# HikariTJU/LD

Hardware: AMD Instinct MI355X
Metric: images/sec (1333x800) GFocal-R50<-R101 LD train step (higher is better)
Workload: dtype f32

## Files before the change

ld_amd/csrc/conv.hip:

```cpp
#include <hip/hip_runtime.h>
#include <type_traits>
#include <stdio.h>
#include <stdlib.h>

#include <mutex>
#include <string>
#include <unordered_map>
#include <vector>

#include "conv_common.h"
#include "conv_tune.h"

namespace {

template <int BM, int BNT, int BKT, int MODE, int KG, int WVM, int WVN>
__global__ __launch_bounds__(64 * WVM * WVN * KG) void conv_igemm_kernel(ConvK a) {
  constexpr int NT = 64 * WVM * WVN;
  constexpr int WM = BM / WVM, WN = BNT / WVN;
  constexpr int TM = WM / 32, TN = WN / 32;
  constexpr int A_PER = BKT * BM / NT;
  constexpr int B_PER = BKT * BNT / NT;
  static_assert(A_PER >= 1 && B_PER >= 1, "tile too small");
  constexpr int NBUF = 2;
  constexpr int GROUP_LDS = NBUF * BKT * (BM + BNT);
  constexpr int NACC = TM * TN * 16;
  static_assert(KG == 1 || (KG - 1) * NACC * NT <= KG * GROUP_LDS,
                "split-K reduction does not fit the tile LDS");
  __shared__ float lds[KG * GROUP_LDS + 2 * BM];
  const int kg = __builtin_amdgcn_readfirstlane((int)threadIdx.x / NT);
  float* As = lds + kg * GROUP_LDS;
  float* Bs = As + NBUF * BKT * BM;

  const int t = threadIdx.x % NT, lane = t & 63, wave = t >> 6;
  const int wm = wave / WVN, wn = wave % WVN;
  const int mtiles = (a.Cout + BM - 1) / BM;
  const int tile = xcd_swizzle(blockIdx.x, gridDim.x);
  const int m0 = (tile % mtiles) * BM;
  const int n0 = (tile / mtiles) * BNT;

  const int jb = n0 + (t % BNT);
  const bool jvalid = jb < a.J;
  int bHin = 0, bWin = 0, boff = 0, bh0 = 0, bw0 = 0;
  if (jvalid) {
    const int n = jb / a.Pout, p = jb - n * a.Pout;
    int bl, bho, bwo;
    locate_out(a.g, p, bl, bho, bwo);
    bHin = a.g.lv[bl].Hin;
    bWin = a.g.lv[bl].Win;
    boff = n * a.Cin * a.Pin + a.g.lv[bl].off_in;
    if (MODE == 1) {
      bh0 = bho + a.ch0;
      bw0 = bwo + a.cw0;
    } else {
      bh0 = bho * a.g.stride - a.g.pad;
      bw0 = bwo * a.g.stride - a.g.pad;
    }
  }
  auto tap_off = [&](int kh, int kw, int& off) -> bool {
    const int hi = bh0 + kh, wi = bw0 + kw;
    if (hi < 0 || hi >= bHin || wi < 0 || wi >= bWin) return false;
    off = boff + hi * bWin + wi;
    return true;
  };
  static_assert(BNT >= 64, "B row groups must be wave-uniform");
  const int bk0 = __builtin_amdgcn_readfirstlane((t / BNT) * B_PER);
  const int am = t % BM;
  const bool avalid = (m0 + am) < a.Cout;
  const int ak0s = __builtin_amdgcn_readfirstlane(((wave * 64) / BM) * A_PER);
  const int ak0v = (BM < 64) ? (lane / BM) * A_PER : 0;
  const int ak0 = ak0s + ak0v;

  floatx16 acc[TM][TN];
#pragma unroll
  for (int i = 0; i < TM; ++i)
#pragma unroll
    for (int j = 0; j < TN; ++j)
#pragma unroll
      for (int r = 0; r < 16; ++r) acc[i][j][r] = 0.0f;

  const int Cin = __builtin_amdgcn_readfirstlane(a.Cin);
  const int Cout = __builtin_amdgcn_readfirstlane(a.Cout);
  const int KW = __builtin_amdgcn_readfirstlane(a.KW);
  const int Pin = __builtin_amdgcn_readfirstlane(a.Pin);
  const int ntaps = __builtin_amdgcn_readfirstlane(
      MODE == 1 ? a.nth * a.ntw : a.KH * a.KW);
  const int csteps = (Cin + BKT - 1) / BKT;
  const int ktot = Cin * ntaps;
  const int nsteps = (MODE == 2) ? (ktot + BKT - 1) / BKT : ntaps * csteps;
  float a_st[A_PER], b_st[B_PER];

  const rsrc_t rx = make_rsrc(a.x, a.x_bytes);
  const rsrc_t rw = make_rsrc(a.wt, a.wt_bytes);
  const int Kpad = __builtin_amdgcn_readfirstlane(a.Kpad);
  const unsigned va =
      avalid ? (unsigned)(m0 + am + ak0v * Cout) * 4u : kOOB;
  auto load_tile = [&](int step, float* ra, float* rb) {
    if (MODE == 2) {
      const int k0 = step * BKT;
#pragma unroll
      for (int i = 0; i < A_PER; ++i)
        ra[i] = buf_load(rw, va, (unsigned)(k0 + ak0s + i) * Cout * 4u);
#pragma unroll
      for (int i = 0; i < B_PER; ++i) {
        const int k = k0 + bk0 + i;
        const int ci = min(k / ntaps, Cin - 1);
        const int r = k % ntaps;
        const int kh = r / KW, kw = r - kh * KW;
        int off = 0;
        const bool kb = jvalid && tap_off(kh, kw, off);
        rb[i] = buf_load(rx, kb ? (unsigned)off * 4u : kOOB,
                           (unsigned)ci * Pin * 4u);
      }
      return;
    }
    int tap = step / csteps;
    const int ci0 = (step - tap * csteps) * BKT;
    int kh, kw;
    if (MODE == 1) {
      const int ntw = __builtin_amdgcn_readfirstlane(a.ntw);
      kh = tap / ntw;
      kw = tap - kh * ntw;
      tap = (a.kh0 + 2 * kh) * KW + a.kw0 + 2 * kw;
    } else {
      kh = tap / KW;
      kw = tap - kh * KW;
    }
    int off = 0;
    const bool ok = jvalid && tap_off(kh, kw, off);
    const unsigned vb = ok ? (unsigned)off * 4u : kOOB;
    const unsigned sa = (unsigned)(tap * Kpad + ci0 + ak0s) * Cout * 4u;
#pragma unroll
    for (int i = 0; i < A_PER; ++i)
      ra[i] = buf_load(rw, va, sa + (unsigned)i * Cout * 4u);
#pragma unroll
    for (int i = 0; i < B_PER; ++i) {
      const int row = min(ci0 + bk0 + i, Cin - 1);
      rb[i] = buf_load(rx, vb, (unsigned)row * Pin * 4u);
    }
  };
  auto store_tile = [&](int buf, const float* ra, const float* rb) {
    float* ap = As + buf * BKT * BM + ak0 * BM + am;
#pragma unroll
    for (int i = 0; i < A_PER; ++i) ap[i * BM] = ra[i];
    float* bp = Bs + buf * BKT * BNT + bk0 * BNT + (t % BNT);
#pragma unroll
    for (int i = 0; i < B_PER; ++i) bp[i * BNT] = rb[i];
  };

  const int l31 = lane & 31, lk = lane >> 5;
  constexpr int KP = BKT / 2;
  auto compute = [&](int buf) {
    const float* ap = As + buf * BKT * BM + wm * WM + l31;
    const float* bp = Bs + buf * BKT * BNT + wn * WN + l31;
    float af[2][TM], bf[2][TN];
#pragma unroll
    for (int i = 0; i < TM; ++i) af[0][i] = ap[lk * BM + i * 32];
// ... 37 lines not shown
      for (int i = 0; i < TM; ++i) f0a[i] = ap[lk * BM + i * 32];
#pragma unroll
      for (int j = 0; j < TN; ++j) f0b[j] = bp[lk * BNT + j * 32];
    };
    auto pstep = [&](int buf, bool has_next, const float* wa, const float* wb) {
      const float* ap = As + buf * BKT * BM + wm * WM + l31;
      const float* bp = Bs + buf * BKT * BNT + wn * WN + l31;
      float af[2][TM], bf[2][TN];
#pragma unroll
      for (int i = 0; i < TM; ++i) af[0][i] = f0a[i];
#pragma unroll
      for (int j = 0; j < TN; ++j) bf[0][j] = f0b[j];
#pragma unroll
      for (int kp = 0; kp < KP; ++kp) {
        const int c = kp & 1;
        if (kp + 1 < KP) {
          const int kr = 2 * (kp + 1) + lk;
#pragma unroll
          for (int i = 0; i < TM; ++i) af[c ^ 1][i] = ap[kr * BM + i * 32];
#pragma unroll
          for (int j = 0; j < TN; ++j) bf[c ^ 1][j] = bp[kr * BNT + j * 32];
        }
        if (kp == WPOS && has_next) store_tile(buf ^ 1, wa, wb);
        if (kp == KP - 2) {
          __syncthreads();
          if (has_next) frag0(buf ^ 1);
        }
        __builtin_amdgcn_sched_barrier(0);
#pragma unroll
        for (int i = 0; i < TM; ++i)
#pragma unroll
          for (int j = 0; j < TN; ++j)
            acc[i][j] = __builtin_amdgcn_mfma_f32_32x32x2f32(af[c][i], bf[c][j],
                                                             acc[i][j], 0, 0, 0);
        __builtin_amdgcn_sched_barrier(0);
      }
    };
    load_tile(0, a_st, b_st);
    store_tile(0, a_st, b_st);
    if (nsteps > 1) load_tile(1, a_s2, b_s2);
    __syncthreads();
    frag0(0);
    for (int step = 0; step < nsteps; step += 2) {
      if (step + 2 < nsteps) load_tile(step + 2, a_st, b_st);
      pstep(0, step + 1 < nsteps, a_s2, b_s2);
      if (step + 1 < nsteps) {
        if (step + 3 < nsteps) load_tile(step + 3, a_s2, b_s2);
        pstep(1, step + 2 < nsteps, a_st, b_st);
      }
    }
  } else {
  const int iters = (nsteps + KG - 1) / KG;
  if (kg < nsteps) {
    load_tile(kg, a_st, b_st);
    store_tile(0, a_st, b_st);
  }
  __syncthreads();
  for (int it = 0; it < iters; ++it) {
    const int cur = it & 1;
    const int step = kg + it * KG;
    const bool more = step + KG < nsteps;
    if (more) load_tile(step + KG, a_st, b_st);
    if (step < nsteps) compute(cur);
    if (more) store_tile(cur ^ 1, a_st, b_st);
    __syncthreads();
  }
  }
  __syncthreads();

  float* s_scale = lds + KG * GROUP_LDS;
  float* s_shift = s_scale + BM;
  if (KG > 1 && kg > 0) {
    float* red = lds + (size_t)(kg - 1) * NACC * NT + t;
#pragma unroll
    for (int i = 0; i < TM; ++i)
#pragma unroll
      for (int j = 0; j < TN; ++j)
#pragma unroll
        for (int r = 0; r < 16; ++r)
          red[((i * TN + j) * 16 + r) * NT] = acc[i][j][r];
  }
  if (kg == 0 && t < BM) {
    const int co = m0 + t;
    float sc = 1.0f, sh = 0.0f;
    if (co < a.Cout) {
      if (a.scale) {
        sc = a.scale[co];
        sh = a.shift[co];
      }
      if (a.bias) sh += a.bias[co];
    }
    s_scale[t] = sc;
    s_shift[t] = sh;
  }
  __syncthreads();
  if (KG > 1) {
    if (kg > 0) return;
#pragma unroll
    for (int g = 1; g < KG; ++g) {
      const float* red = lds + (size_t)(g - 1) * NACC * NT + t;
#pragma unroll
      for (int i = 0; i < TM; ++i)
#pragma unroll
        for (int j = 0; j < TN; ++j)
#pragma unroll
          for (int r = 0; r < 16; ++r)
            acc[i][j][r] += red[((i * TN + j) * 16 + r) * NT];
    }
  }
  const bool has_res = a.residual != nullptr;
  const bool relu = a.relu != 0;
#pragma unroll
  for (int j = 0; j < TN; ++j) {
    const int jc = n0 + wn * WN + j * 32 + l31;
    if (jc >= a.J) continue;
    const int n = jc / a.Pout;
    int p = jc - n * a.Pout;
    int prow = a.Pout;
    if (MODE == 1) {
      int l, hc, wc;
      locate_out(a.g, p, l, hc, wc);
      p = a.foff[l] + (2 * hc + a.ph) * a.fW[l] + 2 * wc + a.pw;
      prow = a.Pfull;
    }
    const size_t colbase = (size_t)n * a.Cout * prow + p;
#pragma unroll
    for (int i = 0; i < TM; ++i) {
      const int rbase = wm * WM + i * 32 + 4 * lk;
      float res[16];
      if (has_res) {
#pragma unroll
        for (int r = 0; r < 16; ++r) {
          const int row = rbase + (r & 3) + 8 * (r >> 2);
          res[r] = (m0 + row < a.Cout)
                       ? a.residual[colbase + (size_t)(m0 + row) * prow]
                       : 0.0f;
        }
      }
#pragma unroll
      for (int r = 0; r < 16; ++r) {
        const int row = rbase + (r & 3) + 8 * (r >> 2);
        if (m0 + row >= a.Cout) continue;
        float v = acc[i][j][r] * s_scale[row] + s_shift[row];
        if (MODE == 0 && a.y_raw)
          a.y_raw[colbase + (size_t)(m0 + row) * prow] = acc[i][j][r];
        if (has_res) v += res[r];
        if (relu) v = fmaxf(v, 0.0f);
        a.y[colbase + (size_t)(m0 + row) * prow] = v;
      }
    }
  }
}

template <int TM, int TN, int WVM, int MODE, int D, int OCC, int KS, int DBG = 0>
__global__ __launch_bounds__(256, OCC) void conv_stream_kernel(ConvK a) {
  static_assert(KS == 1 || (KS == 4 && WVM == 1), "KS is 1 or 4");
  static_assert(D * (TM + TN) < 64, "ring exceeds the 6-bit vmcnt counter");
  constexpr int WVN = 4 / WVM;
  constexpr int WM = TM * 32, WN = TN * 32;
  constexpr int BM = KS == 4 ? WM : WVM * WM, BNT = KS == 4 ? WN : WVN * WN;
  __shared__ float red[KS == 4 ? 2 * TM * TN * 16 * 64 : 1];
  const int lane = threadIdx.x & 63;
  const int wave = __builtin_amdgcn_readfirstlane((int)threadIdx.x >> 6);
  const int wm = KS == 4 ? 0 : wave / WVN, wn = KS == 4 ? 0 : wave % WVN;
  const int kslice = KS == 4 ? wave : 0;
  const int l31 = lane & 31, lk = lane >> 5;
  const int mtiles = (a.Cout + BM - 1) / BM;
  const int tile = xcd_swizzle(blockIdx.x, gridDim.x);
  const int m0 = (tile % mtiles) * BM + wm * WM;
  const int n0 = (tile / mtiles) * BNT + wn * WN;
  if (m0 >= a.Cout || n0 >= a.J) return;

  const int Cin = __builtin_amdgcn_readfirstlane(a.Cin);
  const int Cout = __builtin_amdgcn_readfirstlane(a.Cout);
  const int KW = __builtin_amdgcn_readfirstlane(a.KW);
  const int Pin = __builtin_amdgcn_readfirstlane(a.Pin);
  const int Kpad = __builtin_amdgcn_readfirstlane(a.Kpad);
  const int ntw = __builtin_amdgcn_readfirstlane(MODE == 1 ? a.ntw : a.KW);
  const int ntaps = __builtin_amdgcn_readfirstlane(
      MODE == 1 ? a.nth * a.ntw : a.KH * a.KW);

  int bHin[TN], bWin[TN], boff[TN], bh0[TN], bw0[TN];
#pragma unroll
  for (int j = 0; j < TN; ++j) {
    const int jb = n0 + j * 32 + l31;
    bHin[j] = 0;
    bWin[j] = 0;
    boff[j] = 0;
    bh0[j] = 0;
    bw0[j] = 0;
    if (jb < a.J) {
      const int n = jb / a.Pout, p = jb - n * a.Pout;
      int bl, bho, bwo;
      locate_out(a.g, p, bl, bho, bwo);
      bHin[j] = a.g.lv[bl].Hin;
      bWin[j] = a.g.lv[bl].Win;
      boff[j] = n * Cin * Pin + a.g.lv[bl].off_in + lk * Pin;
      if (MODE == 1) {
        bh0[j] = bho + a.ch0;
        bw0[j] = bwo + a.cw0;
      } else {
        bh0[j] = bho * a.g.stride - a.g.pad;
        bw0[j] = bwo * a.g.stride - a.g.pad;
      }
    }
  }
  unsigned va[TM];
#pragma unroll
  for (int i = 0; i < TM; ++i) {
    const int co = m0 + i * 32 + l31;
    va[i] = co < Cout ? (unsigned)(lk * Cout + co) * 4u : kOOB;
  }
  const rsrc_t rx = make_rsrc(a.x, a.x_bytes);
  const rsrc_t rw = make_rsrc(a.wt, a.wt_bytes);

  unsigned vb[TN];
  int wtap = 0;
  auto set_tap = [&](int tap) {
    int kh = tap / ntw, kw = tap - kh * ntw;
    if (MODE == 1) {
      wtap = (a.kh0 + 2 * kh) * KW + a.kw0 + 2 * kw;
    } else {
      wtap = tap;
    }
#pragma unroll
    for (int j = 0; j < TN; ++j) {
      const int hi = bh0[j] + kh, wi = bw0[j] + kw;
      const bool ok = hi >= 0 && hi < bHin[j] && wi >= 0 && wi < bWin[j];
      vb[j] = ok ? (unsigned)(boff[j] + hi * bWin[j] + wi) * 4u : kOOB;
    }
  };
  float ra[D][TM], rb[D][TN];
  auto load_kp = [&](int d, unsigned sa, unsigned sb) {
#pragma unroll
    for (int i = 0; i < TM; ++i) ra[d][i] = buf_load(rw, (DBG & 4) ? kOOB : va[i], sa);
#pragma unroll
    for (int j = 0; j < TN; ++j) rb[d][j] = buf_load(rx, (DBG & 2) ? kOOB : vb[j], sb);
  };

  floatx16 acc[TM][TN];
#pragma unroll
  for (int i = 0; i < TM; ++i)
#pragma unroll
    for (int j = 0; j < TN; ++j)
#pragma unroll
      for (int r = 0; r < 16; ++r) acc[i][j][r] = 0.0f;
  auto mfma_kp = [&](int d) {
#pragma unroll
    for (int i = 0; i < TM; ++i)
#pragma unroll
      for (int j = 0; j < TN; ++j)
        acc[i][j] = __builtin_amdgcn_mfma_f32_32x32x2f32(ra[d][i], rb[d][j],
                                                         acc[i][j], 0, 0, 0);
  };

  const int cchunks = Cin / (2 * D);
  const int nchunks = ntaps * cchunks;
  const int mychunks = nchunks > kslice ? (nchunks - kslice + KS - 1) / KS : 0;
  int ltap = 0, lci = 0;
  auto advance = [&](int n) {
    lci += 2 * D * n;
    const int t0 = ltap;
    while (lci >= Cin) {
      lci -= Cin;
      ++ltap;
    }
    if (ltap != t0 && ltap < ntaps) set_tap(ltap);
  };
  set_tap(0);
  if (KS > 1) advance(kslice);
  if (mychunks > 0) {
    {
      const unsigned sa = (unsigned)(wtap * Kpad + lci) * Cout * 4u;
      const unsigned sb = (unsigned)lci * Pin * 4u;
#pragma unroll
      for (int d = 0; d < D; ++d) {
        load_kp(d, sa + (unsigned)(2 * d) * Cout * 4u,
                sb + (unsigned)(2 * d) * Pin * 4u);
        __builtin_amdgcn_sched_barrier(0);
      }
      advance(KS);
    }
    for (int c = 0; c + 1 < mychunks; ++c) {
      const unsigned sa = (unsigned)(wtap * Kpad + lci) * Cout * 4u;
      const unsigned sb = (unsigned)lci * Pin * 4u;
#pragma unroll
      for (int d = 0; d < D; ++d) {
        mfma_kp(d);
        __builtin_amdgcn_sched_barrier(0);
        if (!(DBG & 1))
          load_kp(d, sa + (unsigned)(2 * d) * Cout * 4u,
                  sb + (unsigned)(2 * d) * Pin * 4u);
        __builtin_amdgcn_sched_barrier(0);
      }
      advance(KS);
    }
#pragma unroll
    for (int d = 0; d < D; ++d) mfma_kp(d);
  }
  if (KS == 4) {
    constexpr int NACC = TM * TN * 16;
    auto put = [&](float* dst) {
#pragma unroll
      for (int i = 0; i < TM; ++i)
#pragma unroll
        for (int j = 0; j < TN; ++j)
#pragma unroll
          for (int r = 0; r < 16; ++r)
            dst[((i * TN + j) * 16 + r) * 64 + lane] = acc[i][j][r];
    };
    auto add = [&](const float* src) {
#pragma unroll
      for (int i = 0; i < TM; ++i)
#pragma unroll
        for (int j = 0; j < TN; ++j)
#pragma unroll
          for (int r = 0; r < 16; ++r)
            acc[i][j][r] += src[((i * TN + j) * 16 + r) * 64 + lane];
    };
    if (wave >= 2) put(red + (size_t)(wave - 2) * NACC * 64);
    __syncthreads();
    if (wave < 2) add(red + (size_t)wave * NACC * 64);
    __syncthreads();
    if (wave == 1) put(red);
    __syncthreads();
    if (wave != 0) return;
    add(red);
  }

  if (DBG & 8) {
    float s = 0.0f;
#pragma unroll
    for (int i = 0; i < TM; ++i)
#pragma unroll
      for (int j = 0; j < TN; ++j)
#pragma unroll
        for (int r = 0; r < 16; ++r) s += acc[i][j][r];
    if (s == 1.2345e-30f) a.y[0] = s;
    return;
  }
  const bool has_res = a.residual != nullptr;
  const bool has_raw = MODE == 0 && a.y_raw != nullptr;
  const bool relu = a.relu != 0;
  const bool has_aff = a.scale != nullptr, has_bias = a.bias != nullptr;
  const int prow = __builtin_amdgcn_readfirstlane(MODE == 1 ? a.Pfull : a.Pout);
  const unsigned ybytes = (unsigned)a.N * (unsigned)Cout * (unsigned)prow * 4u;
  const rsrc_t r_y = make_rsrc(a.y, ybytes);
  const rsrc_t r_raw = make_rsrc(a.y_raw, has_raw ? ybytes : 0u);
  const rsrc_t r_res = make_rsrc(a.residual, has_res ? ybytes : 0u);
  const rsrc_t r_sc = make_rsrc(a.scale, has_aff ? (unsigned)Cout * 4u : 0u);
  const rsrc_t r_sh = make_rsrc(a.shift, has_aff ? (unsigned)Cout * 4u : 0u);
  const rsrc_t r_bi = make_rsrc(a.bias, has_bias ? (unsigned)Cout * 4u : 0u);
  unsigned voff[TN];
#pragma unroll
  for (int j = 0; j < TN; ++j) {
    const int jc = n0 + j * 32 + l31;
    const int n = jc / a.Pout;
    int p = jc - n * a.Pout;
    if (MODE == 1 && jc < a.J) {
      int l, hc, wc;
      locate_out(a.g, p, l, hc, wc);
      p = a.foff[l] + (2 * hc + a.ph) * a.fW[l] + 2 * wc + a.pw;
    }
    voff[j] = jc < a.J ? ((unsigned)(n * Cout + m0 + 4 * lk) * (unsigned)prow + (unsigned)p) * 4u
                       : kOOB;
  }
  const unsigned prow4 = (unsigned)prow * 4u;
  auto run = [&](auto res_c, auto raw_c) {
    constexpr bool RES = decltype(res_c)::value, RAW = decltype(raw_c)::value;
#pragma unroll
    for (int ig = 0; ig < TM * 4; ++ig) {
      const int i = ig >> 2, g = ig & 3;
      const int rl = i * 32 + 8 * g;
      __builtin_amdgcn_sched_barrier(0);
      float sc[4], sh[4], bi[4], rv[TN][4];
#pragma unroll
      for (int e = 0; e < 4; ++e) {
        const unsigned ro = (unsigned)(m0 + 4 * lk + rl + e) * 4u;
        sc[e] = buf_load(r_sc, ro, 0);
        sh[e] = buf_load(r_sh, ro, 0);
        bi[e] = buf_load(r_bi, ro, 0);
      }
      if (RES) {
#pragma unroll
        for (int j = 0; j < TN; ++j)
#pragma unroll
          for (int e = 0; e < 4; ++e) {
            const bool ok = m0 + 4 * lk + rl + e < Cout;
            rv[j][e] = buf_load(r_res, ok ? voff[j] : kOOB, (unsigned)(rl + e) * prow4);
          }
      }
#pragma unroll
      for (int e = 0; e < 4; ++e) {
        const bool ok = m0 + 4 * lk + rl + e < Cout;
        const float scale = has_aff ? sc[e] : 1.0f;
        const float shift = sh[e] + bi[e];
        const unsigned so = (unsigned)(rl + e) * prow4;
#pragma unroll
        for (int j = 0; j < TN; ++j) {
          const int r = 4 * g + e;
          const unsigned vo = ok ? voff[j] : kOOB;
          const float av = acc[i][j][r];
          float v = av * scale + shift;
          if (RAW)
            __builtin_amdgcn_raw_buffer_store_b32(__builtin_bit_cast(unsigned, av), r_raw,
                                                  vo, so, 0);
          if (RES) v += rv[j][e];
          v = relu ? fmaxf(v, 0.0f) : v;
          __builtin_amdgcn_raw_buffer_store_b32(__builtin_bit_cast(unsigned, v), r_y, vo,
                                                so, 0);
        }
      }
    }
  };
  if (has_res) {
    if (has_raw) run(std::true_type{}, std::true_type{});
    else run(std::true_type{}, std::false_type{});
  } else {
    if (has_raw) run(std::false_type{}, std::true_type{});
    else run(std::false_type{}, std::false_type{});
  }
}

template <int VEC>
struct VecF;
template <>
struct VecF<2> { typedef float T __attribute__((ext_vector_type(2))); };
template <>
struct VecF<4> { typedef float T __attribute__((ext_vector_type(4))); };

template <int VEC>
__device__ __forceinline__ typename VecF<VEC>::T buf_load_vec(rsrc_t r, unsigned voff,
                                                             unsigned soff) {
  typedef typename VecF<VEC>::T V;
  if constexpr (VEC == 2)
    return __builtin_bit_cast(V, __builtin_amdgcn_raw_buffer_load_b64(r, voff, soff, 0));
  else
    return __builtin_bit_cast(V, __builtin_amdgcn_raw_buffer_load_b128(r, voff, soff, 0));
}

template <int TM, int VEC, int WVM, int D>
__global__ __launch_bounds__(256, 2) void conv1x1_vec_kernel(ConvK a) {
  static_assert(D * (TM + 1) < 64, "ring exceeds the 6-bit vmcnt counter");
  typedef typename VecF<VEC>::T V;
  constexpr int WVN = 4 / WVM;
  constexpr int WM = TM * 32, WN = VEC * 32;
  constexpr int BM = WVM * WM, BNT = WVN * WN;
  const int lane = threadIdx.x & 63;
  const int wave = __builtin_amdgcn_readfirstlane((int)threadIdx.x >> 6);
  const int wm = wave / WVN, wn = wave % WVN;
  const int l31 = lane & 31, lk = lane >> 5;
// ... 756 lines not shown
    s += *reinterpret_cast<const floatx4*>(slabs + (size_t)k * per + i);
  if (ntaps == 1) {
    float* o = dw + (size_t)co * Cin + ci;
    if (accumulate) s += *reinterpret_cast<const floatx4*>(o);
    *reinterpret_cast<floatx4*>(o) = s;
  } else {
#pragma unroll
    for (int e = 0; e < 4; ++e) {
      const size_t o = ((size_t)co * Cin + ci + e) * ntaps + tap;
      dw[o] = accumulate ? dw[o] + s[e] : s[e];
    }
  }
}

__device__ __forceinline__ void weight_transform_at(const float* __restrict__ w,
                                                    int Cout, int Cin, int ntaps,
                                                    int CinPad, int CoutPad,
                                                    float* __restrict__ wt_fwd,
                                                    float* __restrict__ wt_bwd,
                                                    size_t i) {
  if (wt_fwd && i < (size_t)ntaps * CinPad * Cout) {
    const int co = (int)(i % Cout);
    const size_t q = i / Cout;
    const int ci = (int)(q % CinPad), tap = (int)(q / CinPad);
    wt_fwd[i] = ci < Cin ? w[((size_t)co * Cin + ci) * ntaps + tap] : 0.0f;
  }
  if (wt_bwd && i < (size_t)ntaps * CoutPad * Cin) {
    const int ci = (int)(i % Cin);
    const size_t q = i / Cin;
    const int co = (int)(q % CoutPad), tapf = (int)(q / CoutPad);
    wt_bwd[i] = co < Cout
                    ? w[((size_t)co * Cin + ci) * ntaps + (ntaps - 1 - tapf)]
                    : 0.0f;
  }
}

__global__ void conv_weight_transform_kernel(const float* __restrict__ w, int Cout,
                                             int Cin, int ntaps, int CinPad,
                                             int CoutPad,
                                             float* __restrict__ wt_fwd,
                                             float* __restrict__ wt_bwd) {
  weight_transform_at(w, Cout, Cin, ntaps, CinPad, CoutPad, wt_fwd, wt_bwd,
                      (size_t)blockIdx.x * blockDim.x + threadIdx.x);
}

__global__ __launch_bounds__(256) void conv_weight_transform_batch_kernel(
    const ld_wt_job_t* __restrict__ jobs, const int32_t* __restrict__ block_job) {
  const ld_wt_job_t j = jobs[block_job[blockIdx.x]];
  const int CinPad = (j.Cin + kKPad - 1) / kKPad * kKPad;
  const int CoutPad = (j.Cout + kKPad - 1) / kKPad * kKPad;
  weight_transform_at(j.w, j.Cout, j.Cin, j.ntaps, CinPad, CoutPad, j.wt_fwd, j.wt_bwd,
                      (size_t)(blockIdx.x - j.first_block) * 256 + threadIdx.x);
}

int check_conv(const ld_conv_t* c) {
  if (!c || c->N < 1 || c->Cin < 1 || c->Cout < 1 || c->KH < 1 || c->KW < 1 ||
      c->num_levels < 1 || c->num_levels > LD_MAX_LEVELS)
    return LD_EINVAL;
  if (c->stride != 1 && c->stride != 2) return LD_EUNSUPPORTED;
  int pin = 0, pout = 0;
  for (int l = 0; l < c->num_levels; ++l) {
    const ld_conv_level_t& v = c->lv[l];
    if (v.off_in != pin || v.off_out != pout) return LD_EINVAL;
    if ((v.Hin + 2 * c->pad - c->KH) / c->stride + 1 != v.Hout ||
        (v.Win + 2 * c->pad - c->KW) / c->stride + 1 != v.Wout)
      return LD_EINVAL;
    pin += v.Hin * v.Win;
    pout += v.Hout * v.Wout;
  }
  if (pin != c->Pin || pout != c->Pout) return LD_EINVAL;
  return 0;
}

struct TileCfg { int bm, bn, bk; };

inline int tile_blocks(const ConvK& k, const TileCfg& c) {
  return ((k.Cout + c.bm - 1) / c.bm) * ((k.J + c.bn - 1) / c.bn);
}

inline TileCfg pick_tile(const ConvK& k) {
  if (const char* env = getenv("LD_CONV_TILE")) {
    TileCfg c{0, 0, 0};
    if (sscanf(env, "%dx%dx%d", &c.bm, &c.bn, &c.bk) == 3) return c;
  }
  const int ktot = k.Cin * k.KH * k.KW;
  return TileCfg{64, 64, ktot >= 512 ? 32 : 16};
}

inline int set_extents(ConvK& k, size_t x_floats, size_t wt_floats) {
  const size_t y_floats = (size_t)k.N * k.Cout * (size_t)max(k.Pout, k.Pfull);
  if (x_floats * 4 >= (size_t)kOOB || wt_floats * 4 >= (size_t)kOOB ||
      y_floats * 4 >= (size_t)kOOB)
    return LD_EUNSUPPORTED;
  k.x_bytes = (unsigned)(x_floats * 4);
  k.wt_bytes = (unsigned)(wt_floats * 4);
  return 0;
}

struct StreamCfg {
  int tm, tn, wvm, d, ks;
};
#define LD_STREAM_SHAPES(X)                                                        \
  X(2, 2, 2, 8, 1) X(2, 2, 1, 8, 1) X(2, 1, 2, 8, 1) X(1, 2, 2, 8, 1)              \
  X(1, 2, 4, 8, 1) X(1, 2, 1, 8, 1) X(1, 1, 2, 8, 1) X(1, 1, 1, 8, 1)              \
  X(1, 1, 4, 8, 1) X(3, 1, 1, 8, 1) X(3, 2, 1, 8, 1) X(2, 2, 2, 4, 1)              \
  X(2, 2, 1, 4, 1) X(1, 2, 2, 4, 1) X(1, 1, 2, 4, 1) X(1, 1, 1, 4, 1)              \
  X(3, 1, 1, 4, 1) X(3, 2, 1, 4, 1) X(1, 1, 1, 8, 4) X(1, 2, 1, 8, 4)              \
  X(2, 1, 1, 8, 4) X(2, 2, 1, 8, 4)                                                \
  X(1, 1, 1, 16, 1) X(1, 1, 2, 16, 1) X(1, 1, 4, 16, 1) X(2, 1, 2, 16, 1)          \
  X(1, 2, 2, 16, 1) X(2, 1, 1, 16, 1) X(1, 1, 1, 16, 4) X(2, 1, 1, 16, 4)          \
  X(1, 2, 1, 16, 4)
#define LD_VEC_SHAPES(X)                                                           \
  X(1, 4, 1, 8, 2) X(1, 4, 2, 8, 2) X(1, 4, 4, 8, 2) X(2, 4, 1, 8, 2)              \
  X(2, 4, 2, 8, 2) X(1, 2, 1, 8, 2) X(1, 2, 2, 8, 2) X(1, 2, 4, 8, 2)              \
  X(2, 2, 2, 8, 2) X(1, 4, 2, 16, 2) X(1, 4, 4, 16, 2) X(1, 2, 4, 16, 2)
constexpr StreamCfg kStreamCfgs[] = {
#define LD_STREAM_ROW(TM_, TN_, WVM_, D_, KS_) {TM_, TN_, WVM_, D_, KS_},
    LD_STREAM_SHAPES(LD_STREAM_ROW) LD_VEC_SHAPES(LD_STREAM_ROW)
#undef LD_STREAM_ROW
};
constexpr int kNumStreamCfgs = sizeof(kStreamCfgs) / sizeof(kStreamCfgs[0]);

inline unsigned cap_lds_bytes(int cap, int static_bytes) {
  static const int kb[] = {0, 64, 64, 48, 36, 28, 24};
  if (cap < 2 || cap > 6) return 0;
  const int want = kb[cap] * 1024 - static_bytes;
  return want > 0 ? (unsigned)want : 0;
}

template <int MODE>
int launch_stream_cfg(const ConvK& k, const StreamCfg& c, hipStream_t stream,
                      int cap = 0) {
  if (const char* env = getenv("LD_ALLOW_WRONG_RESULTS") ? getenv("LD_STREAM_DBG") : nullptr) {
    const int dbg = atoi(env);
    if (MODE == 0 && dbg && c.tm == 1 && c.tn == 1 && c.wvm == 1 && c.d == 16) {
      const int bm = 32, bn = 32;
      const int nb = ((k.Cout + bm - 1) / bm) * ((k.J + bn - 1) / bn);
#define LD_DBG_CASE(V_)                                                                  \
  if (dbg == V_ && c.ks == 4) {                                                          \
    LD_LAUNCH((conv_stream_kernel<1, 1, 1, 0, 16, 4, 4, V_>), dim3(nb), dim3(256), \
                       0, stream, k);                                                    \
    return (int)hipGetLastError();                                                       \
  }
      LD_DBG_CASE(1) LD_DBG_CASE(2) LD_DBG_CASE(4) LD_DBG_CASE(6) LD_DBG_CASE(8) LD_DBG_CASE(9)
      LD_DBG_CASE(14)
#undef LD_DBG_CASE
    }
  }
  const int bm = (c.ks == 4 ? 1 : c.wvm) * c.tm * 32;
  const int bn = (c.ks == 4 ? 1 : 4 / c.wvm) * c.tn * 32;
  const int nb = ((k.Cout + bm - 1) / bm) * ((k.J + bn - 1) / bn);
  const unsigned lds =
      cap_lds_bytes(cap, c.ks == 4 ? 2 * c.tm * c.tn * 16 * 64 * 4 : 4);
#define LD_STREAM_CASE(TM_, TN_, WVM_, D_, KS_)                                    \
  if (c.tm == TM_ && c.tn == TN_ && c.wvm == WVM_ && c.d == D_ && c.ks == KS_) {   \
    LD_LAUNCH((conv_stream_kernel<TM_, TN_, WVM_, MODE, D_, (KS_ == 4 ? 4 : 2), KS_>), \
                       dim3(nb), dim3(256), lds, stream, k);                       \
    return (int)hipGetLastError();                                                 \
  }
  if (c.ks != 2) {
    LD_STREAM_SHAPES(LD_STREAM_CASE)
  }
#undef LD_STREAM_CASE
  if constexpr (MODE == 0) {
#define LD_VEC_CASE(TM_, TN_, WVM_, D_, KS_)                                       \
  if (c.ks == 2 && c.tm == TM_ && c.tn == TN_ && c.wvm == WVM_ && c.d == D_) {     \
    LD_LAUNCH((conv1x1_vec_kernel<TM_, TN_, WVM_, D_>), dim3(nb), dim3(256), lds, \
                       stream, k);                                                 \
    return (int)hipGetLastError();                                                 \
  }
    LD_VEC_SHAPES(LD_VEC_CASE)
#undef LD_VEC_CASE
  }
  return LD_EUNSUPPORTED;
}

#define MODE1_TAPS(k) ((k).nth > 0 ? (k).nth * (k).ntw : (k).KH * (k).KW)
inline bool stream_cfg_fits(const ConvK& k, const StreamCfg& c) {
  if (c.wvm < 1) return false;
  if (k.Cin % (2 * c.d) != 0) return false;
  if (c.ks == 2) {
    if (k.KH != 1 || k.KW != 1 || k.g.stride != 1 || k.g.pad != 0 || k.nth > 0 ||
        k.Pin != k.Pout || k.Pout % c.tn != 0 || k.x_c8 || k.y_c8 || k.res_c8)
      return false;
    const uintptr_t m = (uintptr_t)(c.tn * 4 - 1);
    if ((((uintptr_t)k.x | (uintptr_t)k.y | (uintptr_t)k.residual |
          (uintptr_t)k.y_raw) & m) != 0)
      return false;
    const int bmv = c.wvm * c.tm * 32, cout32v = (k.Cout + 31) / 32 * 32;
    if (c.wvm > 1 && bmv > cout32v) return false;
    if (c.wvm == 1 && c.tm * 32 >= cout32v + 32) return false;
    return true;
  }
  if (c.d == 4 && k.Cin % 16 == 0) return false;
  const int bm = c.wvm * c.tm * 32;
  const int cout32 = (k.Cout + 31) / 32 * 32;
  if (c.ks == 4) {
    const int nchunks = (MODE1_TAPS(k)) * (k.Cin / (2 * c.d));
    if (nchunks < 16) return false;
  }
  if (c.wvm > 1 && bm > cout32) return false;
  if (c.wvm == 1 && c.tm * 32 >= cout32 + 32) return false;
  return true;
}

inline int stream_cfg_model(const ConvK& k) {
  int best = -1;
  double best_t = 0;
  for (int i = 0; i < kNumStreamCfgs; ++i) {
    const StreamCfg& c = kStreamCfgs[i];
    if (c.ks == 2) continue;
    if (!stream_cfg_fits(k, c)) continue;
    const int bm = (c.ks == 4 ? 1 : c.wvm) * c.tm * 32;
    const int bn = (c.ks == 4 ? 1 : 4 / c.wvm) * c.tn * 32;
    const long nb = (long)((k.Cout + bm - 1) / bm) * ((k.J + bn - 1) / bn);
    const int area = c.tm * c.tn;
    const double eff = (area >= 4 ? 0.90 : area >= 2 ? 0.84 : 0.79) *
                       (c.ks == 4 ? 0.97 : 1.0);
    const int occ = area >= 4 ? 4 : 5;
    const double rounds =
        nb <= 256L * occ ? (double)((nb + 255) / 256) : (double)nb / 256.0;
    const double t = rounds * (c.ks == 4 ? 1 : 4) * area / eff;
    if (best < 0 || t < best_t) {
      best = i;
      best_t = t;
    }
  }
  return best;
}

inline LdTuneCfg stream_cfg_rec(const StreamCfg& c) {
  return LdTuneCfg{c.tm, c.tn, c.wvm, c.d, c.ks};
}

template <int MODE>
int launch_stream(const ConvK& k, hipStream_t stream) {
  if (k.Cin % 8 != 0) return LD_EUNSUPPORTED;
  auto launch = [&](const StreamCfg& c, int cap) {
    return launch_stream_cfg<MODE>(k, c, stream, cap);
  };
  auto by_model = [&] {
    const int m = stream_cfg_model(k);
    return m < 0 ? LD_EUNSUPPORTED : launch(kStreamCfgs[m], 0);
  };
  auto forced = [&](int* rc) {
    const char* env = getenv("LD_CONV_STREAM");
    if (!env) return false;
    *rc = LD_EUNSUPPORTED;
    if (env[0] == '0' && env[1] == 0) return true;
    StreamCfg c;
    c.ks = 1;
    int cap = 0;
    if (sscanf(env, "%dx%dx%dx%dx%dx%d", &c.tm, &c.tn, &c.wvm, &c.d, &c.ks, &cap) < 4)
      return false;
    while (c.d > 4 && k.Cin % (2 * c.d) != 0) c.d /= 2;
    if (!(c.ks == 2 && !stream_cfg_fits(k, c))) {
      *rc = launch(c, cap);
      if (*rc != LD_EUNSUPPORTED) return true;
      c.ks = 1;
      *rc = launch(c, cap);
      if (*rc != LD_EUNSUPPORTED) return true;
    }
    *rc = by_model();
    return true;
  };
  return launch_picked(MODE, 0, k, kStreamCfgs, forced, stream_cfg_rec, stream_cfg_fits,
                       stream_cfg_model, launch);
}

template <int MODE>
int tune_stream(const ConvK& k, hipStream_t stream) {
  if (k.Cin % 8 != 0) return 1;
  const LdTuneKey key = make_tune_key(MODE, 0, k);
  if (int r = tune_refused(key, stream)) return r;
  int pick = stream_cfg_model(k);
  if (pick < 0) return 1;
  TuneTimer timer(stream);
  float best_ms = -1.0f;
  int best_cap = 0;
  static const int kCaps[] = {0, 4, 3, 2};
  for (int i = 0; i < kNumStreamCfgs; ++i) {
    if (!stream_cfg_fits(k, kStreamCfgs[i])) continue;
    for (const int cap_try : kCaps) {
      const float ms = timer.time(
          [&] { return launch_stream_cfg<MODE>(k, kStreamCfgs[i], stream, cap_try); });
      if (ms == TuneTimer::kLaunchFailed) break;
      if (ms < 0.0f) continue;
      if (best_ms < 0.0f || ms < best_ms * (cap_try ? 0.99f : 1.0f)) {
        best_ms = ms;
        pick = i;
        best_cap = cap_try;
      }
    }
  }
  const StreamCfg& c = kStreamCfgs[pick];
  if (tune_log_level() == 1) {
    const double fl = 2.0 * k.J * k.Cout * k.Cin *
                      (MODE == 1 ? k.nth * k.ntw : k.KH * k.KW);
    fprintf(stderr,
            "[ld_conv] mode %d Cin %d Cout %d k %dx%d s%d J %d lv %d -> "
            "%dx%dx%dx%dx%d cap %d  %.1f TFLOP/s\n",
            MODE, k.Cin, k.Cout, k.KH, k.KW, k.g.stride, k.J, k.g.num_levels,
            c.tm, c.tn, c.wvm, c.d, c.ks, best_cap, tune_tflops(fl, best_ms));
  }
  if (best_ms > 0.0f) {
    LdTuneCfg rec = stream_cfg_rec(c);
    rec.cap = best_cap;
    ld_tune_store(key, rec);
// ... 956 lines not shown
```

Baseline: 58.62.

## Replace KS=4 split-K chain reduction with two-stage butterfly LDS combine and buffer-store epilogue

For the split-K-by-4 stream conv kernel, the four waves now combine partial accumulators with a two-step pairwise exchange through LDS. Each step swaps half of the remaining values, so every wave ends up owning a quarter of the output rows and writes them itself, instead of reducing through a serial chain. Output-channel lanes are XOR-swizzled per wave so that each wave's owned rows line up. The epilogue now uses buffer loads and stores with prefetched scale, shift, bias and residual, and is specialised on the residual and raw flags. The old chain path stays reachable through an environment variable, but this adds register pressure and more complex indexing.

```diff
diff --git a/ld_amd/csrc/conv.hip b/ld_amd/csrc/conv.hip
--- a/ld_amd/csrc/conv.hip
+++ b/ld_amd/csrc/conv.hip
@@ -2,6 +2,7 @@
 #include <type_traits>
 #include <stdio.h>
 #include <stdlib.h>
+#include <string.h>
 
 #include <mutex>
 #include <string>
@@ -345,14 +346,118 @@
   }
 }
 
-template <int TM, int TN, int WVM, int MODE, int D, int OCC, int KS, int DBG = 0>
+template <int TN>
+struct StreamEp {
+  bool has_res, has_raw, relu, has_aff;
+  rsrc_t r_y, r_raw, r_res, r_sc, r_sh, r_bi;
+  unsigned voff[TN], prow4;
+};
+template <int TN, int MODE>
+__device__ __forceinline__ StreamEp<TN> stream_ep(const ConvK& a, int Cout, int m0, int n0,
+                                                  int lk, int l31) {
+  StreamEp<TN> E;
+  E.has_res = a.residual != nullptr;
+  E.has_raw = MODE == 0 && a.y_raw != nullptr;
+  E.relu = a.relu != 0;
+  E.has_aff = a.scale != nullptr;
+  const bool has_bias = a.bias != nullptr;
+  const int prow = __builtin_amdgcn_readfirstlane(MODE == 1 ? a.Pfull : a.Pout);
+  const unsigned ybytes = (unsigned)a.N * (unsigned)Cout * (unsigned)prow * 4u;
+  E.r_y = make_rsrc(a.y, ybytes);
+  E.r_raw = make_rsrc(a.y_raw, E.has_raw ? ybytes : 0u);
+  E.r_res = make_rsrc(a.residual, E.has_res ? ybytes : 0u);
+  E.r_sc = make_rsrc(a.scale, E.has_aff ? (unsigned)Cout * 4u : 0u);
+  E.r_sh = make_rsrc(a.shift, E.has_aff ? (unsigned)Cout * 4u : 0u);
+  E.r_bi = make_rsrc(a.bias, has_bias ? (unsigned)Cout * 4u : 0u);
+#pragma unroll
+  for (int j = 0; j < TN; ++j) {
+    const int jc = n0 + j * 32 + l31;
+    const int n = jc / a.Pout;
+    int p = jc - n * a.Pout;
+    if (MODE == 1 && jc < a.J) {
+      int l, hc, wc;
+      locate_out(a.g, p, l, hc, wc);
+      p = a.foff[l] + (2 * hc + a.ph) * a.fW[l] + 2 * wc + a.pw;
+    }
+    E.voff[j] = jc < a.J ? ((unsigned)(n * Cout + m0 + 4 * lk) * (unsigned)prow + (unsigned)p) * 4u
+                         : kOOB;
+  }
+  E.prow4 = (unsigned)prow * 4u;
+  return E;
+}
+template <int TN>
+struct StreamGroupOps {
+  float sc[4], sh[4], bi[4], rv[TN][4];
+};
+template <int TN>
+__device__ __forceinline__ void stream_group_res(const StreamEp<TN>& E, StreamGroupOps<TN>& o,
+                                                 int Cout, int row0, int rl) {
+#pragma unroll
+  for (int j = 0; j < TN; ++j)
+#pragma unroll
+    for (int e = 0; e < 4; ++e) {
+      const bool ok = row0 + rl + e < Cout;
+      o.rv[j][e] = buf_load(E.r_res, ok ? E.voff[j] : kOOB, (unsigned)(rl + e) * E.prow4);
+    }
+}
+template <int TN, class ResC>
+__device__ __forceinline__ void stream_group_loads(ResC, const StreamEp<TN>& E,
+                                                   StreamGroupOps<TN>& o, int Cout, int row0,
+                                                   int rl) {
+#pragma unroll
+  for (int e = 0; e < 4; ++e) {
+    const unsigned ro = (unsigned)(row0 + rl + e) * 4u;
+    o.sc[e] = buf_load(E.r_sc, ro, 0);
+    o.sh[e] = buf_load(E.r_sh, ro, 0);
+    o.bi[e] = buf_load(E.r_bi, ro, 0);
+  }
+  if (ResC::value) stream_group_res<TN>(E, o, Cout, row0, rl);
+}
+template <int TN>
+__device__ __forceinline__ void stream_group_affine(const StreamEp<TN>& E,
+                                                    StreamGroupOps<TN>& o) {
+#pragma unroll
+  for (int e = 0; e < 4; ++e) {
+    o.sc[e] = E.has_aff ? o.sc[e] : 1.0f;
+    o.sh[e] = o.sh[e] + o.bi[e];
+  }
+}
+template <int TN, class ResC, class RawC>
+__device__ __forceinline__ void stream_group_stores(ResC, RawC, const StreamEp<TN>& E,
+                                                    const StreamGroupOps<TN>& o,
+                                                    const float (&acc4)[TN][4], int Cout,
+                                                    int row0, int rl) {
+#pragma unroll
+  for (int e = 0; e < 4; ++e) {
+    const bool ok = row0 + rl + e < Cout;
+    const unsigned so = (unsigned)(rl + e) * E.prow4;
+#pragma unroll
+    for (int j = 0; j < TN; ++j) {
+      const unsigned vo = ok ? E.voff[j] : kOOB;
+      const float av = acc4[j][e];
+      float v = av * o.sc[e] + o.sh[e];
+      if (RawC::value)
+        __builtin_amdgcn_raw_buffer_store_b32(__builtin_bit_cast(unsigned, av), E.r_raw, vo,
+                                              so, 0);
+      if (ResC::value) v += o.rv[j][e];
+      v = E.relu ? fmaxf(v, 0.0f) : v;
+      __builtin_amdgcn_raw_buffer_store_b32(__builtin_bit_cast(unsigned, v), E.r_y, vo, so, 0);
+    }
+  }
+}
+
+constexpr int kStreamW4 = 16;
+template <int TM, int TN, int WVM, int MODE, int D, int OCC, int KS, int FLAGS = 0>
 __global__ __launch_bounds__(256, OCC) void conv_stream_kernel(ConvK a) {
+  constexpr int DBG = FLAGS & 15;
+  constexpr bool W4 = (FLAGS & kStreamW4) != 0;
   static_assert(KS == 1 || (KS == 4 && WVM == 1), "KS is 1 or 4");
+  static_assert(!W4 || (KS == 4 && DBG == 0), "W4 is a KS = 4 tail");
   static_assert(D * (TM + TN) < 64, "ring exceeds the 6-bit vmcnt counter");
   constexpr int WVN = 4 / WVM;
   constexpr int WM = TM * 32, WN = TN * 32;
   constexpr int BM = KS == 4 ? WM : WVM * WM, BNT = KS == 4 ? WN : WVN * WN;
-  __shared__ float red[KS == 4 ? 2 * TM * TN * 16 * 64 : 1];
+  __shared__ alignas(16) float red[KS == 4 ? 2 * TM * TN * 16 * 64 : 1];
   const int lane = threadIdx.x & 63;
   const int wave = __builtin_amdgcn_readfirstlane((int)threadIdx.x >> 6);
   const int wm = KS == 4 ? 0 : wave / WVN, wn = KS == 4 ? 0 : wave % WVN;
@@ -401,7 +506,7 @@
   unsigned va[TM];
 #pragma unroll
   for (int i = 0; i < TM; ++i) {
-    const int co = m0 + i * 32 + l31;
+    const int co = m0 + i * 32 + (W4 ? l31 ^ (8 * wave) : l31);
     va[i] = co < Cout ? (unsigned)(lk * Cout + co) * 4u : kOOB;
   }
   const rsrc_t rx = make_rsrc(a.x, a.x_bytes);
@@ -490,6 +595,87 @@
     }
 #pragma unroll
     for (int d = 0; d < D; ++d) mfma_kp(d);
+  }
+  if constexpr (W4) {
+    const int lane = __builtin_amdgcn_mbcnt_hi(~0u, __builtin_amdgcn_mbcnt_lo(~0u, 0u));
+    const int l31 = lane & 31, lk = lane >> 5;
+    const StreamEp<TN> E = stream_ep<TN, MODE>(a, Cout, m0, n0, lk, l31);
+    constexpr int NT = TM * TN, BOX = NT * 2 * 64;
+    floatx4* const box = reinterpret_cast<floatx4*>(red);
+    __builtin_amdgcn_sched_barrier(0);
+    StreamGroupOps<TN> o[TM];
+    stream_group_loads<TN>(std::false_type{}, E, o[0], Cout, m0 + 4 * lk, 8 * wave);
+    if (E.has_res) stream_group_res<TN>(E, o[0], Cout, m0 + 4 * lk, 8 * wave);
+    __builtin_amdgcn_sched_barrier(0);
+    float keep[NT][2][4];
+    {
+      floatx4* const out = box + (wave ^ 2) * BOX + lane;
+#pragma unroll
+      for (int t = 0; t < NT; ++t)
+#pragma unroll
+        for (int q = 0; q < 2; ++q) {
+          floatx4 v;
+#pragma unroll
+          for (int e = 0; e < 4; ++e) v[e] = acc[t / TN][t % TN][8 + 4 * q + e];
+          out[(t * 2 + q) * 64] = v;
+        }
+      __syncthreads();
+      const floatx4* const in = box + wave * BOX + lane;
+#pragma unroll
+      for (int t = 0; t < NT; ++t)
+#pragma unroll
+        for (int q = 0; q < 2; ++q) {
+          const floatx4 v = in[(t * 2 + q) * 64];
+#pragma unroll
+          for (int e = 0; e < 4; ++e) keep[t][q][e] = acc[t / TN][t % TN][4 * q + e] + v[e];
+        }
+    }
+    stream_group_affine<TN>(E, o[0]);
+    __builtin_amdgcn_sched_barrier(0);
+    float own[NT][4];
+    {
+      floatx4* const out = box + wave * BOX + lane;
+#pragma unroll
+      for (int t = 0; t < NT; ++t) {
+        floatx4 v;
+#pragma unroll
+        for (int e = 0; e < 4; ++e) v[e] = keep[t][1][e];
+        out[t * 64] = v;
+      }
+      __syncthreads();
+      const floatx4* const in = box + (wave ^ 1) * BOX + lane;
+#pragma unroll
+      for (int t = 0; t < NT; ++t) {
+        const floatx4 v = in[t * 64];
+#pragma unroll
+        for (int e = 0; e < 4; ++e) own[t][e] = keep[t][0][e] + v[e];
+      }
+    }
+    auto tail = [&](auto res_c, auto raw_c) {
+#pragma unroll
+      for (int i = 0; i < TM; ++i) {
+        if (i + 1 < TM)
+          stream_group_loads<TN>(res_c, E, o[i + 1], Cout, m0 + 4 * lk,
+                                 (i + 1) * 32 + 8 * wave);
+        if (i > 0) stream_group_affine<TN>(E, o[i]);
+        float av[TN][4];
+#pragma unroll
+        for (int j = 0; j < TN; ++j)
+#pragma unroll
+          for (int e = 0; e < 4; ++e) av[j][e] = own[i * TN + j][e];
+        stream_group_stores<TN>(res_c, raw_c, E, o[i], av, Cout, m0 + 4 * lk,
+                                i * 32 + 8 * wave);
+        __builtin_amdgcn_sched_barrier(0);
+      }
+    };
+    if (E.has_res) {
+      if (E.has_raw) tail(std::true_type{}, std::true_type{});
+      else tail(std::true_type{}, std::false_type{});
+    } else {
+      if (E.has_raw) tail(std::false_type{}, std::true_type{});
+      else tail(std::false_type{}, std::false_type{});
+    }
+    return;
   }
   if (KS == 4) {
     constexpr int NACC = TM * TN * 16;
@@ -1552,8 +1738,17 @@
   const int nb = ((k.Cout + bm - 1) / bm) * ((k.J + bn - 1) / bn);
   const unsigned lds =
       cap_lds_bytes(cap, c.ks == 4 ? 2 * c.tm * c.tn * 16 * 64 * 4 : 4);
+  const char* comb = getenv("LD_CONV_KS4_COMBINE");
+  const bool chain = comb && strcmp(comb, "chain") == 0;
 #define LD_STREAM_CASE(TM_, TN_, WVM_, D_, KS_)                                    \
   if (c.tm == TM_ && c.tn == TN_ && c.wvm == WVM_ && c.d == D_ && c.ks == KS_) {   \
+    if constexpr (KS_ == 4) {                                                      \
+      if (!chain) {                                                                \
+        LD_LAUNCH((conv_stream_kernel<TM_, TN_, 1, MODE, D_, 4, 4, kStreamW4>), dim3(nb),  \
+                  dim3(256), lds, stream, k);                                      \
+        return (int)hipGetLastError();                                             \
+      }                                                                            \
+    }                                                                              \
     LD_LAUNCH((conv_stream_kernel<TM_, TN_, WVM_, MODE, D_, (KS_ == 4 ? 4 : 2), KS_>), \
                        dim3(nb), dim3(256), lds, stream, k);                       \
     return (int)hipGetLastError();                                                 \
```

Measured after the change: 57.70. 0.984x the previous value.
